# ImIntheMiddle/VATL4Pose-WACV2024

Measured on AMD Instinct MI355X. Metric: frames/sec pose-infer+uncertainty, 256x192 17-kp, higher is better.
Workload: dtype f32; 1 GPU; SimpleBaseline-R50 256x192 inference + decode + local-peak + THC-L1, 1024-frame synthetic video per GPU; frames_per_gpu=1024, batch=1024, tracks=4, parallelism=frame-sharded x1

## Files before the change

include/vatl_hip.h:

```cpp
#ifndef VATL_HIP_H
#define VATL_HIP_H

#include <stdint.h>

#ifdef __cplusplus
extern "C" {
#endif

#define VATL_VERSION 100
#define VATL_EINVAL  (-1)
#define VATL_ELAUNCH (-2)

int         vatl_version(void);
const char* vatl_last_error(void);

int vatl_flop_meter_begin(void);
int vatl_flop_meter_end(double* direct_flops, double* winograd_flops, int64_t* direct_launches, int64_t* winograd_launches);
#define VATL_ROUTE_NAMES "igemm,igemm_bnbwd,igemm_dma,persistent_1x1,streamk,rows_1x1,bottleneck_chain,stem_pool,halo_3x3," \
                         "winograd,winograd_2h,winograd_bnbwd,winograd_persist,winograd_c32,wgrad,winograd_wgrad,winograd_wgrad_2h," \
                         "winograd_wgrad_table,winograd_f4,winograd_f4_bnbwd,gemm1x1_ring,winograd_deconv43,winograd_s2_43,stem_pool_w1d," \
                         "chain_proj,chain_step,gemm1x1_bf16x6"
int vatl_flop_meter_routes(int64_t* counts, int n);


int vatl_nchw_to_nhwc(const float* src, float* dst, int N, int C, int H, int W, int Cpad, void* stream);
int vatl_nhwc_to_nchw(const float* src, float* dst, int N, int C, int H, int W, void* stream);

int vatl_pack_conv_weight(const float* w_oihw, float* w_packed, int Cout, int Cin, int R, int S,
                          int CoutPad, int Spad, int CinPad, void* stream);
int vatl_pack_deconv4x4s2_weight(const float* w_iohw, float* w_packed, int Cin, int Cout, int CoutPad, void* stream);
int64_t vatl_stem_pool_weight_floats(void);
int vatl_pack_stem_pool_weight(const float* w_oihw, float* packed, void* stream);
int vatl_stem_pool_supported(int H, int W);
int vatl_stem7x7s2_pool_fwd(const float* x_nchw, const float* w_packed, const float* scale, const float* bias, float* y_nhwc,
                            int N, int H, int W, void* stream);
int64_t vatl_stem_pool_w1d_weight_floats(void);
// ... 309 lines not shown
int vatl_deconv4x4s2_winograd43_supported(int N, int H, int W, int Cin, int Cout);
int vatl_deconv4x4s2_winograd43_fwd(const float* x, const float* u, const float* scale, const float* bias, float* y, int N, int H, int W,
                                    int Cin, int Cout, int relu, void* stream);
int64_t vatl_winograd_s2_43_weight_floats(int Cout, int Cin);
int vatl_pack_winograd_s2_43_weight(const float* w, float* u, int Cout, int Cin, void* stream);
int vatl_conv3x3s2_winograd43_supported(int N, int H, int W, int Cin, int Cout);
int vatl_conv3x3s2_winograd43_fwd(const float* x, const float* u, const float* scale, const float* bias, float* y, int N, int H, int W,
                                  int Cin, int Cout, int relu, void* stream);
int64_t vatl_gemm1x1_bf16x6_weight_floats(int N, int K);
int vatl_pack_gemm1x1_bf16x6_weight(const float* w, float* u, int N, int K, void* stream);
int vatl_gemm1x1_bf16x6_supported(int64_t M, int K, int K1, int N);
int vatl_gemm1x1_bf16x6_fwd(const float* x, const float* u, const float* scale, const float* bias, const float* residual, float* y,
                            int N, int H, int W, int Cin, int Cout, int stride, int relu, void* stream);
int vatl_gemm1x1_bf16x6_dual_fwd(const float* a, const float* x, const float* u, const float* bias, const float* residual, float* y,
                                 int N, int Ho, int Wo, int C1, int H2, int W2, int C2, int stride2, int Cout, int relu, void* stream);
int64_t vatl_winograd_deconv_stats_row_blocks(int64_t N, int H, int W);
int vatl_deconv4x4s2_winograd_fwd_stats(const float* x, const float* u, float* y, double* stats, int64_t* row_blocks_used, int N, int H, int W,
                                        int Cin, int Cout, void* stream);
int64_t vatl_conv3x3_winograd_wgrad_workspace_floats(int Cout, int Cin, int64_t N, int H, int W);
int vatl_conv3x3_winograd_wgrad(const float* x, const float* dz, float* dw, float* workspace, int N, int H, int W, int Cin, int Cout, void* stream);
int64_t vatl_deconv4x4s2_winograd_wgrad_workspace_floats(int Cin, int Cout, int64_t N, int H, int W);
int vatl_deconv4x4s2_winograd_wgrad(const float* x, const float* dy, float* dw, float* workspace, int N, int H, int W, int Cin, int Cout,
                                    void* stream);
int64_t vatl_winograd_deconv_dgrad_weight_floats(int Cin, int Cout);
int vatl_pack_winograd_deconv_dgrad_weight(const float* w, float* u, int Cin, int Cout, void* stream);
int vatl_deconv4x4s2_winograd_dgrad(const float* dz, const float* u, const float* residual, float* dx, int N, int H, int W, int Cin, int Cout,
                                    void* stream);
int vatl_deconv4x4s2_winograd_dgrad_bnbwd(const float* dz, const float* u, const float* residual, float* dx, int N, int H, int W, int Cin,
                                          int Cout, const float* bn_z, const float* bn_mask_y, const float* bn_scale, const float* bn_bias,
                                          const float* bn_mean, const float* bn_invstd, double* stats, int64_t* row_blocks_used, void* stream);
// ... 82 lines not shown
```

vatl4pose-wacv2024_amd/alphapose/models/hip_engine.py:

```python
from __future__ import annotations

import time
import weakref

import torch
import torch.nn as nn

import vatl_hip as vh

MAX_CHUNK = 1024



WINOGRAD = True
ROWS_GEMM = True
ROWS_GEMM_K = (128, 256)
WINO_C32 = True
WINO_F4 = True
DECONV_43 = True
S2_43 = True
BF16X6 = True


class _Conv:
    __slots__ = ("w", "u", "u32", "u4", "us2", "ux6", "wsrc", "wino", "c32", "f4", "s2", "x6", "scale", "bias", "cout", "r", "s", "stride", "pad")

    def __init__(self, conv: nn.Conv2d, bn: nn.BatchNorm2d | None):
        assert conv.groups == 1 and conv.dilation == (1, 1)
        assert conv.stride[0] == conv.stride[1] and conv.padding[0] == conv.padding[1]
        self.w = vh.pack_conv_weight(conv.weight.detach())
        self.cout, _, self.r, self.s = conv.weight.shape
        self.stride, self.pad = conv.stride[0], conv.padding[0]
        self.u = self.u32 = self.u4 = None
        self.wino = WINOGRAD and (self.r, self.s, self.stride, self.pad) == (3, 3, 1, 1) and conv.in_channels % 16 == 0 and self.cout % 4 == 0
        self.c32 = self.wino and WINO_C32 and conv.in_channels == 32 and self.cout == 32
        self.f4 = self.wino and WINO_F4 and conv.in_channels >= 64 and conv.in_channels % 16 == 0 and self.cout % 64 == 0
        self.us2 = None
        self.s2 = WINOGRAD and S2_43 and (self.r, self.s, self.stride, self.pad) == (3, 3, 2, 1) and conv.in_channels % 16 == 0 and self.cout % 64 == 0
        self.ux6 = None
        self.x6 = (BF16X6 and (self.r, self.s, self.stride, self.pad) == (1, 1, 1, 0) and conv.in_channels >= 512 and conv.in_channels % 64 == 0
                   and self.cout % 128 == 0)
        self.wsrc = conv.weight.detach() if self.wino or self.s2 else None
        cb =conv.bias.detach() if conv.bias is not None else None
        if bn is not None:
            self.scale, self.bias = vh.bn_fold(_d(bn.weight), _d(bn.bias), bn.running_mean, bn.running_var, bn.eps, cb)
        elif cb is not None:
            self.scale, self.bias = vh.bn_fold(None, None, None, None, 0.0, cb, channels=self.cout)
        else:
            self.scale = self.bias = None

    def __call__(self, x, relu, residual=None, out_nchw=False, out=None):
        if self.wino and not out_nchw and not vh.latency_mode():
            if self.c32 and vh.conv3x3_winograd_c32_supported(x.shape[0], x.shape[1], x.shape[2], 32, 32):
                if self.u32 is None:
                    self.u32 = vh.pack_winograd_c32_weight(self.wsrc)
                return vh.conv3x3_winograd_c32_fwd(x, self.u32, self.scale, self.bias, relu, residual=residual, out=out)
            if self.f4 and vh.conv3x3_winograd_f4_supported(x.shape[0], x.shape[1], x.shape[2], x.shape[3], self.cout):
                if self.u4 is None:
                    self.u4 = vh.pack_winograd_f4_weight(self.wsrc)
                return vh.conv3x3_winograd_f4_fwd(x, self.u4, self.scale, self.bias, self.cout, relu, residual=residual, out=out)
            if self.u is None:
                self.u = vh.pack_winograd_weight(self.wsrc)
            return vh.conv3x3_winograd_fwd(x, self.u, self.scale, self.bias, self.cout, relu, residual=residual, out=out)
        if (ROWS_GEMM and self.r == 1 and self.stride == 1 and not out_nchw and not vh.latency_mode() and x.shape[-1] in ROWS_GEMM_K
                and vh.conv1x1_rows_supported(x.shape[-1], 0, self.cout, x.shape[0] * x.shape[1] * x.shape[2])):
            return vh.conv1x1_rows_fwd(x, self.w, self.scale, self.bias, self.cout, relu, residual=residual, out=out)
        us2 = None
        if self.s2 and residual is None and not out_nchw and not vh.latency_mode():
            if self.us2 is None and vh.conv3x3s2_winograd43_supported(x.shape[0], x.shape[1], x.shape[2], x.shape[3], self.cout):
                self.us2 = vh.pack_winograd_s2_43_weight(self.wsrc)
            us2 = self.us2
        ux6 = None
        if self.x6 and not out_nchw and not vh.latency_mode():
            if self.ux6 is None and vh.gemm1x1_bf16x6_supported(x.shape[0] * x.shape[1] * x.shape[2], x.shape[3], 0, self.cout):
                self.ux6 = vh.pack_gemm1x1_bf16x6_weight(self.w)
            ux6 = self.ux6
        return vh.conv2d_fwd(x, self.w, self.scale, self.bias, self.cout, self.r, self.s, self.stride, self.pad, relu,
                             residual=residual, out_nchw=out_nchw, out=out, u_s2=us2, u_x6=ux6)
# ... 562 lines not shown
```

vatl4pose-wacv2024_amd/csrc/common.h:

```cpp
#pragma once
#include <hip/hip_runtime.h>
#include <atomic>
#include <cstdarg>
#include <cstdio>
#include <cstdint>

#include "vatl_hip.h"

namespace vatl {

char* err_buf();
int fail(int code, const char* fmt, ...);

void meter_add(int kind, double flops);
enum MeterRoute {
    kRouteIgemm = 0, kRouteIgemmBnBwd, kRouteIgemmDma, kRoutePersistent1x1, kRouteStreamK, kRouteRows, kRouteChain, kRouteStemPool, kRouteHalo,
    kRouteWino, kRouteWino2H, kRouteWinoBnBwd, kRouteWinoPersist, kRouteWinoC32, kRouteWgrad, kRouteWinoWgrad, kRouteWinoWgrad2H,
    kRouteWinoWgradTable, kRouteWinoF4, kRouteWinoF4BnBwd, kRouteGemm1x1Ring, kRouteWinoDeconv43, kRouteWinoS2_43, kRouteStemPoolW1d, kRouteChainProj,
    kRouteChainStep, kRouteGemm1x1Bf16x6, kRouteCount
};
void meter_route(int route);

inline int check_launch(const char* what) {
    hipError_t e = hipGetLastError();
    if (e != hipSuccess) return fail(VATL_ELAUNCH, "%s: %s", what, hipGetErrorString(e));
    return 0;
}

inline int ensure_dynamic_lds(const void* kern, int bytes, std::atomic<unsigned>& done_mask, const char* what) {
    int d = 0;
    if (hipGetDevice(&d) != hipSuccess) return fail(VATL_ELAUNCH, "%s: no current device", what);
    const unsigned bit = 1u << (d & 31);
    if (done_mask.load(std::memory_order_acquire) & bit) return 0;
    hipError_t e = hipFuncSetAttribute(kern, hipFuncAttributeMaxDynamicSharedMemorySize, bytes);
// ... 59 lines not shown
```

vatl4pose-wacv2024_amd/csrc/gemm1x1_bf16x6.hip:

```cpp
#include "conv_igemm.h"
#include "split16.h"
#include "tile_order.h"

namespace vatl {

constexpr int X6_BK = 16;
constexpr int X6_NS = 4;
constexpr int X6_A_FLOATS = 128 * X6_BK;
constexpr int X6_B_BYTES = 3 * 128 * X6_BK * 2;
constexpr int X6_STAGE = X6_A_FLOATS + X6_B_BYTES / 4;
constexpr int X6_BYTES = X6_NS * X6_STAGE * (int)sizeof(float);

typedef __bf16 x6_bf16x8 __attribute__((ext_vector_type(8)));

template <int N>
__device__ __forceinline__ void x6_wait_vm() {
    static_assert(N == 0 || N == 5 || N == 10, "add the count here");
    if constexpr (N == 0) asm volatile("s_waitcnt vmcnt(0)" ::: "memory");
    else if constexpr (N == 5) asm volatile("s_waitcnt vmcnt(5)" ::: "memory");
    else asm volatile("s_waitcnt vmcnt(10)" ::: "memory");
}

__device__ __forceinline__ f32x16 x6_mfma(u32x4 a, u32x4 b, f32x16 c) {
    return __builtin_amdgcn_mfma_f32_32x32x16_bf16(__builtin_bit_cast(x6_bf16x8, a), __builtin_bit_cast(x6_bf16x8, b), c, 0, 0, 0);
}

template <bool DUAL, bool RES>
__device__ __forceinline__ void gemm1x1_bf16x6_body(const ConvParams& p, float* smem) {
    const int tid = threadIdx.x, lane = tid & 63;
    const int wave = __builtin_amdgcn_readfirstlane(tid >> 6);
    const int wm = wave >> 1, wn = wave & 1;

    const int t = xcd_contiguous_index(blockIdx.x, gridDim.x);
    const int m_tile = t / p.n_tiles, n_tile = t - m_tile * p.n_tiles;
    const int m0 = m_tile * 128, n0 = n_tile * 128;

    const __amdgpu_buffer_rsrc_t xr = buf_rsrc(p.x, p.x_bytes);
    const __amdgpu_buffer_rsrc_t wr = buf_rsrc(p.w, p.w_bytes);
    const __amdgpu_buffer_rsrc_t xr2 = buf_rsrc(DUAL ? p.x2 : p.x, DUAL ? p.x2_bytes : p.x_bytes);

    const int S = p.ktiles * 2;
    const int S1 = DUAL ? p.k1 * 2 : S;

// ... 23 lines not shown
            if constexpr (DUAL && decltype(src)::value == 1) __builtin_amdgcn_raw_ptr_buffer_load_lds(xr2, da, 16, aoff2[u], (unsigned)(s - S1) * 64u, 0, 0);
            else                                             __builtin_amdgcn_raw_ptr_buffer_load_lds(xr, da, 16, aoff[u], (unsigned)s * 64u, 0, 0);
        }
#pragma unroll
        for (int u = 0; u < 3; ++u)
            __builtin_amdgcn_raw_ptr_buffer_load_lds(wr, (lds_void*)(st + X6_A_FLOATS + (4 * u + wave) * 256), 16, boff[u], (unsigned)s * (unsigned)X6_B_BYTES, 0, 0);
    };

    const int frow = lane & 31, h = lane >> 5;
    const int fsw = (frow >> 2) & 3;
    const float* Ard[2];
#pragma unroll
    for (int c = 0; c < 2; ++c) Ard[c] = smem + (wm * 64 + frow) * X6_BK + (((2 * h + c) ^ fsw) << 2);
    const float* Brd = smem + X6_A_FLOATS + (2 * wn * 64 + lane) * 4;

    f32x16 acc[2][2], sml[2][2];
#pragma unroll
    for (int i = 0; i < 2; ++i)
#pragma unroll
        for (int j = 0; j < 2; ++j)
#pragma unroll
            for (int e = 0; e < 16; ++e) { acc[i][j][e] = 0.f; sml[i][j][e] = 0.f; }

    auto stage = [&](auto slot, auto kind, auto src, int s) {
        constexpr int B = decltype(slot)::value, KIND = decltype(kind)::value;
        if constexpr (KIND <= 1) x6_wait_vm<10>();
        else if constexpr (KIND == 2) x6_wait_vm<5>();
        else x6_wait_vm<0>();
        __builtin_amdgcn_s_barrier();
        asm volatile("" ::: "memory");
        f32x4 af[2][2];
        u32x4 bw[3][2];
#pragma unroll
        for (int i = 0; i < 2; ++i)
#pragma unroll
            for (int c = 0; c < 2; ++c) af[i][c] = *reinterpret_cast<const f32x4*>(Ard[c] + B * X6_STAGE + i * 32 * X6_BK);
#pragma unroll
        for (int pl = 0; pl < 3; ++pl)
#pragma unroll
            for (int j = 0; j < 2; ++j) bw[pl][j] = *reinterpret_cast<const u32x4*>(Brd + B * X6_STAGE + (4 * pl + j) * 256);
        if constexpr (KIND == 0) issue(src, (B + 3) & 3, s + 3);
        u32x4 a0[2], a1[2], a2[2];
#pragma unroll
        for (int i = 0; i < 2; ++i)
#pragma unroll
            for (int d = 0; d < 4; ++d) {
                const split16::Pieces e = split16::split3(af[i][d >> 1][(2 * d) & 3]), o = split16::split3(af[i][d >> 1][(2 * d + 1) & 3]);
                a0[i][d] = split16::pack_pair(e.hi, o.hi);
                a1[i][d] = split16::pack_pair(e.mid, o.mid);
                a2[i][d] = split16::pack_pair(e.lo, o.lo);
            }
#pragma unroll
        for (int i = 0; i < 2; ++i)
#pragma unroll
            for (int j = 0; j < 2; ++j) acc[i][j] = x6_mfma(a0[i], bw[0][j], acc[i][j]);
#pragma unroll
// ... 37 lines not shown
    int s = 0;
    if constexpr (DUAL) {
        for (; s < S1 - 4; s += 4) group(C0{}, s);
        stage(C0{}, C0{}, C0{}, s);
        stage(C1{}, C0{}, X2{}, s + 1);
        stage(C2{}, C0{}, X2{}, s + 2);
        stage(C3{}, C0{}, X2{}, s + 3);
        s += 4;
    }
    for (; s < S - 4; s += 4) group(X2{}, s);
    stage(C0{}, C0{}, X2{}, s);
    stage(C1{}, C1{}, X2{}, s + 1);
    stage(C2{}, C2{}, X2{}, s + 2);
    stage(C3{}, C3{}, X2{}, s + 3);

    const unsigned rowb = (unsigned)p.Cout * 4u;
    const unsigned ylane = (unsigned)(m0 + wm * 64 + 4 * h) * rowb + (unsigned)(n0 + wn * 64 + frow) * 4u;
    const __amdgpu_buffer_rsrc_t yr = buf_rsrc(p.y, p.y_bytes);
    const __amdgpu_buffer_rsrc_t rr = buf_rsrc(RES ? p.res : p.y, RES ? p.y_bytes : 0u);
    float sc[2], bi[2];
#pragma unroll
    for (int j = 0; j < 2; ++j) {
        const int n = n0 + wn * 64 + j * 32 + frow;
        sc[j] = p.scale ? p.scale[n] : 1.f;
        bi[j] = p.bias ? p.bias[n] : 0.f;
    }
    const float lo = p.relu ? 0.f : -INFINITY;
#pragma unroll
    for (int i = 0; i < 2; ++i) {
        float rs[2][16];
#pragma unroll
        for (int j = 0; j < 2; ++j)
#pragma unroll
            for (int e = 0; e < 16; ++e)
                rs[j][e] = RES ? buf_load1(rr, ylane + (unsigned)(32 * i + (e & 3) + 8 * (e >> 2)) * rowb + (unsigned)j * 128u) : 0.f;
#pragma unroll
        for (int j = 0; j < 2; ++j)
#pragma unroll
            for (int e = 0; e < 16; ++e) {
                const float a = acc[i][j][e] + sml[i][j][e];
                const float v = fmaxf(a * sc[j] + bi[j] + rs[j][e], lo);
                buf_store1(yr, ylane + (unsigned)(32 * i + (e & 3) + 8 * (e >> 2)) * rowb + (unsigned)j * 128u, v);
            }
    }
}

template <bool DUAL, bool RES>
__global__ __launch_bounds__(256, 2) void gemm1x1_bf16x6_kernel(ConvParams p) {
    extern __shared__ __attribute__((aligned(16))) float smem[];
    gemm1x1_bf16x6_body<DUAL, RES>(p, smem);
}

__global__ __launch_bounds__(256) void gemm1x1_bf16x6_pack_kernel(const float* __restrict__ w, u32x4* __restrict__ u, int K, long long units) {
    const long long idx = (long long)blockIdx.x * 256 + threadIdx.x;
    if (idx >= units) return;
    const int S = K / X6_BK;
    const int l = (int)(idx & 63), jb = (int)((idx >> 6) & 3);
    const long long rest = idx >> 8;
    const int pl = (int)(rest % 3);
    const long long ts = rest / 3;
    const int st = (int)(ts % S), n_tile = (int)(ts / S);
    const float* src = w + (long long)(n_tile * 128 + jb * 32 + (l & 31)) * K + st * X6_BK + 8 * (l >> 5);
    float pc[8];
#pragma unroll
    for (int j = 0; j < 8; ++j) {
// ... 1 lines not shown
        pc[j] = pl == 0 ? q.hi : (pl == 1 ? q.mid : q.lo);
    }
    u32x4 o;
#pragma unroll
    for (int d = 0; d < 4; ++d) o[d] = split16::pack_pair(pc[2 * d], pc[2 * d + 1]);
    u[idx] = o;
}

static bool x6_shape_ok(long long M, int K, int K1, int N) {
    if (M < 1 || N < 128 || (N % 128) || K < 1 || (K % 64)) return false;
    if (K1 == 0 ? K < 512 : (K1 < 64 || (K1 % 64) || K - K1 < 64 || K < 384)) return false;
    if ((M + 128) * N >= (1LL << 30) || M * (K1 ? K1 : K) >= (1LL << 30) || 6LL * N * K >= (1LL << 31)) return false;
    return true;
}

template <bool DUAL, bool RES>
static int launch_x6_impl(const ConvParams& p, hipStream_t st) {
    auto kern = gemm1x1_bf16x6_kernel<DUAL, RES>;
    static std::atomic<unsigned> configured{0};
    if (int rc = ensure_dynamic_lds(reinterpret_cast<const void*>(kern), X6_BYTES, configured, "gemm1x1_bf16x6")) return rc;
    ConvParams q = p;
    q.n_tiles = p.Cout / 128;
    q.m_tiles = cdiv(p.M, 128);
    q.splits = 1;
    hipLaunchKernelGGL(kern, dim3((unsigned)(q.m_tiles * q.n_tiles)), dim3(256), X6_BYTES, st, q);
    meter_add(0, (6.0 / 16.0) * 2.0 * ((double)q.m_tiles * 128) * ((double)q.n_tiles * 128) * ((double)q.ktiles * BK));
    meter_route(kRouteGemm1x1Bf16x6);
    return check_launch("gemm1x1_bf16x6");
}

}

using namespace vatl;

extern "C" int64_t vatl_gemm1x1_bf16x6_weight_floats(int N, int K) { return 3LL * N * K / 2; }

extern "C" int vatl_pack_gemm1x1_bf16x6_weight(const float* w, float* u, int N, int K, void* stream) {
    if (!w || !u) return fail(VATL_EINVAL, "pack_gemm1x1_bf16x6_weight: null pointer");
    if (N < 128 || (N % 128) || K < 64 || (K % 64) || 6LL * N * K >= (1LL << 31))
        return fail(VATL_EINVAL, "pack_gemm1x1_bf16x6_weight: N %d must be a multiple of 128, K %d of 64, 6 N K below 2^31 bytes", N, K);
    const long long units = 6LL * N * K / 16;
    hipLaunchKernelGGL(gemm1x1_bf16x6_pack_kernel, dim3((unsigned)((units + 255) / 256)), dim3(256), 0, (hipStream_t)stream, w, reinterpret_cast<u32x4*>(u), K, units);
    return check_launch("gemm1x1_bf16x6_pack");
}

extern "C" int vatl_gemm1x1_bf16x6_supported(int64_t M, int K, int K1, int N) { return x6_shape_ok(M, K, K1, N) ? 1 : 0; }

extern "C" int vatl_gemm1x1_bf16x6_fwd(const float* x, const float* u, const float* scale, const float* bias, const float* residual, float* y,
                                       int N, int H, int W, int Cin, int Cout, int stride, int relu, void* stream) {
    if (!x || !u || !y || N <= 0 || H <= 0 || W <= 0) return fail(VATL_EINVAL, "gemm1x1_bf16x6_fwd: null pointer or empty batch");
    const long long M = (long long)N * H * W;
    if (stride != 1 || !x6_shape_ok(M, Cin, 0, Cout))
        return fail(VATL_EINVAL, "gemm1x1_bf16x6_fwd: %lld x %d -> %d, stride %d is outside stride 1, K %% 64 == 0, K >= 512, N %% 128 == 0 and 32-bit offsets", M, Cin, Cout, stride);
    ConvParams p{};
    p.x = x; p.w = u; p.scale = scale; p.bias = bias; p.res = residual; p.y = y;
    p.N = N; p.H = H; p.W = W; p.Cin = Cin; p.Cout = Cout; p.CoutPad = Cout;
    p.R = 1; p.S = 1; p.stride = 1;
    p.Ho = H; p.Wo = W; p.M = (int)M;
    p.OH = H; p.OW = W; p.osy = 1; p.osx = 1;
    p.relu = relu;
    p.kpr = Cin / BK; p.ktiles = p.kpr; p.K = Cin;
    p.x_bytes = (unsigned)(M * Cin * 4); p.y_bytes = (unsigned)(M * Cout * 4); p.w_bytes = (unsigned)(6LL * Cout * Cin);
    p.d_HoWo = make_fastdiv((unsigned)(H * W)); p.d_Wo = make_fastdiv((unsigned)W);
    return residual ? launch_x6_impl<false, true>(p, (hipStream_t)stream) : launch_x6_impl<false, false>(p, (hipStream_t)stream);
}

extern "C" int vatl_gemm1x1_bf16x6_dual_fwd(const float* a, const float* x, const float* u, const float* bias, const float* residual, float* y,
                                            int N, int Ho, int Wo, int C1, int H2, int W2, int C2, int stride2, int Cout, int relu, void* stream) {
    if (!a || !x || !u || !y || N <= 0 || Ho <= 0 || Wo <= 0) return fail(VATL_EINVAL, "gemm1x1_bf16x6_dual_fwd: null pointer or empty batch");
    if (residual) return fail(VATL_EINVAL, "gemm1x1_bf16x6_dual_fwd: the dual form takes no residual");
    if (stride2 < 1 || (long long)(Ho - 1) * stride2 >= H2 || (long long)(Wo - 1) * stride2 >= W2)
        return fail(VATL_EINVAL, "gemm1x1_bf16x6_dual_fwd: stride %d does not map %dx%d onto %dx%d", stride2, Ho, Wo, H2, W2);
    const long long M = (long long)N * Ho * Wo, x2e = (long long)N * H2 * W2 * C2;
    if (C1 <= 0 || C2 <= 0 || !x6_shape_ok(M, C1 + C2, C1, Cout) || x2e >= (1LL << 30))
        return fail(VATL_EINVAL, "gemm1x1_bf16x6_dual_fwd: %lld x (%d + %d) -> %d is outside C1 %% 64 == 0, C2 %% 64 == 0, K >= 384, N %% 128 == 0 and 32-bit offsets", M, C1, C2, Cout);
    ConvParams p{};
    p.x = a; p.x2 = x; p.w = u; p.bias = bias; p.y = y;
    p.N = N; p.H = Ho; p.W = Wo; p.Cin = C1; p.Cout = Cout; p.CoutPad = Cout;
    p.R = 1; p.S = 1; p.stride = 1;
// ... 10 lines not shown
```

vatl4pose-wacv2024_amd/vatl_hip/__init__.py:

```python
from __future__ import annotations

import ctypes as C
import os
import threading as _threading

import torch

_HERE = os.path.dirname(os.path.abspath(__file__))
LIB_PATH = os.environ.get("VATL_HIP_LIB") or os.path.join(_HERE, "libvatl_hip.so")

_p = C.c_void_p
_i = C.c_int
_f = C.c_float
_d = C.c_double
_i64 = C.c_int64

SIGNATURES = {
    "vatl_version": (_i, []),
    "vatl_last_error": (C.c_char_p, []),
    "vatl_flop_meter_begin": (_i, []),
    "vatl_flop_meter_end": (_i, [_p, _p, _p, _p]),
    "vatl_flop_meter_routes": (_i, [_p, _i]),
    "vatl_nchw_to_nhwc": (_i, [_p, _p, _i, _i, _i, _i, _i, _p]),
    "vatl_nhwc_to_nchw": (_i, [_p, _p, _i, _i, _i, _i, _p]),
# ... 94 lines not shown
    "vatl_pack_winograd_deconv_weight": (_i, [_p, _p, _i, _i, _p]),
    "vatl_deconv4x4s2_winograd_fwd": (_i, [_p] * 5 + [_i] * 6 + [_p]),
    "vatl_winograd_deconv43_weight_floats": (_i64, [_i, _i]),
    "vatl_pack_winograd_deconv43_weight": (_i, [_p, _p, _i, _i, _p]),
    "vatl_deconv4x4s2_winograd43_supported": (_i, [_i, _i, _i, _i, _i]),
    "vatl_deconv4x4s2_winograd43_fwd": (_i, [_p] * 5 + [_i] * 6 + [_p]),
    "vatl_winograd_s2_43_weight_floats": (_i64, [_i, _i]),
    "vatl_pack_winograd_s2_43_weight": (_i, [_p, _p, _i, _i, _p]),
    "vatl_conv3x3s2_winograd43_supported": (_i, [_i, _i, _i, _i, _i]),
    "vatl_conv3x3s2_winograd43_fwd": (_i, [_p] * 5 + [_i] * 6 + [_p]),
    "vatl_gemm1x1_bf16x6_weight_floats": (_i64, [_i, _i]),
    "vatl_pack_gemm1x1_bf16x6_weight": (_i, [_p, _p, _i, _i, _p]),
    "vatl_gemm1x1_bf16x6_supported": (_i, [_i64, _i, _i, _i]),
    "vatl_gemm1x1_bf16x6_fwd": (_i, [_p] * 6 + [_i] * 7 + [_p]),
    "vatl_gemm1x1_bf16x6_dual_fwd": (_i, [_p] * 6 + [_i] * 10 + [_p]),
    "vatl_winograd_deconv_stats_row_blocks": (_i64, [_i64, _i, _i]),
    "vatl_deconv4x4s2_winograd_fwd_stats": (_i, [_p, _p, _p, _p, _p, _i, _i, _i, _i, _i, _p]),
    "vatl_conv2d_fwd_stats": (_i, [_p, _p, _p, _p, _p, _i, _i, _i, _i, _i, _i, _i, _i, _i, _i, _p]),
    "vatl_deconv4x4s2_fwd_stats": (_i, [_p, _p, _p, _p, _p, _i, _i, _i, _i, _i, _i, _p]),
    "vatl_bn_train_finalize": (_i, [_p, _i64, _i64, _i, _p, _p, _p, _p, _f, _f, _p, _p, _p, _p, _p]),
    "vatl_maxpool3x3s2_bwd": (_i, [_p, _p, _p, _i, _i, _i, _i, _p]),
    "vatl_maxpool3x3s2_fwd_idx": (_i, [_p, _p, _p, _i, _i, _i, _i, _p]),
    "vatl_pack_weights_multi": (_i, [_p, _i, _i64, _p]),
    "vatl_adamw_multi_block_elems": (_i64, []),
    "vatl_checksum_block_words": (_i64, []),
    "vatl_checksum_multi": (_i, [_p, _i, _i64, _p, _p]),
    "vatl_maxpool3x3s2_fwd_idx_affine": (_i, [_p, _p, _p, _p, _p, _i, _i, _i, _i, _p]),
    "vatl_bn_train_bwd_relu_pool": (_i, [_p, _p, _p, _p, _p, _p, _p, _p, _p, _p, _p, _i, _i, _i, _i, _p, _p, _p]),
    "vatl_maxpool3x3s2_bwd_idx": (_i, [_p, _p, _p, _i, _i, _i, _i, _p]),
    "vatl_pixelunshuffle2": (_i, [_p, _p, _i, _i, _i, _i, _p]),
# ... 156 lines not shown
    y = torch.empty((n, h, w, cpad), device=x.device, dtype=torch.float32)
    _check(lib().vatl_nchw_to_nhwc(_ptr(x), _ptr(y), n, c, h, w, cpad, _stream()), "vatl_nchw_to_nhwc")
    return y


def nhwc_to_nchw(x: torch.Tensor) -> torch.Tensor:
    n, h, w, c = x.shape
    y = torch.empty((n, c, h, w), device=x.device, dtype=torch.float32)
    _check(lib().vatl_nhwc_to_nchw(_ptr(x), _ptr(y), n, c, h, w, _stream()), "vatl_nhwc_to_nchw")
    return y



ROUTE_NAMES = ("igemm", "igemm_bnbwd", "igemm_dma", "persistent_1x1", "streamk", "rows_1x1", "bottleneck_chain", "stem_pool", "halo_3x3", "winograd",
               "winograd_2h", "winograd_bnbwd", "winograd_persist", "winograd_c32", "wgrad", "winograd_wgrad", "winograd_wgrad_2h", "winograd_wgrad_table", "winograd_f4", "winograd_f4_bnbwd",
               "gemm1x1_ring", "winograd_deconv43", "winograd_s2_43", "stem_pool_w1d", "chain_proj", "chain_step", "gemm1x1_bf16x6")


class flop_meter:

    def __enter__(self):
        _check(lib().vatl_flop_meter_begin(), "flop_meter_begin")
        self.direct = self.winograd = self.total = 0.0
        self.direct_launches = self.winograd_launches = 0
        return self

    @staticmethod
    def launches_now() -> int:
        counts = (C.c_int64 * len(ROUTE_NAMES))()
        _check(min(0, lib().vatl_flop_meter_routes(counts, len(ROUTE_NAMES))), "flop_meter_routes")
        return int(sum(counts))
# ... 352 lines not shown
    scale = torch.empty(c, device=dev, dtype=torch.float32)
    bias = torch.empty(c, device=dev, dtype=torch.float32)
    _check(lib().vatl_bn_fold(_ptr(gamma), _ptr(beta), _ptr(mean), _ptr(var), _ptr(conv_bias), eps, _ptr(scale), _ptr(bias), c, _stream()), "vatl_bn_fold")
    return scale, bias



def conv3x3s2_winograd43_supported(n: int, h: int, w: int, cin: int, cout: int) -> bool:
    return bool(lib().vatl_conv3x3s2_winograd43_supported(n, h, w, cin, cout))


def gemm1x1_bf16x6_supported(m: int, k: int, k1: int, n: int) -> bool:
    return bool(lib().vatl_gemm1x1_bf16x6_supported(m, k, k1, n))


def conv2d_fwd(x, w_packed, scale, bias, cout: int, r: int, s: int, stride: int, pad: int, relu: bool,
               residual=None, out_nchw: bool = False, out=None, u_s2=None, u_x6=None):
    n, h, w, cin = x.shape
    ho = (h + 2 * pad - r) // stride + 1
    wo = (w + 2 * pad - s) // stride + 1
    shape = (n, cout, ho, wo) if out_nchw else (n, ho, wo, cout)
    y = out if out is not None else torch.empty(shape, device=x.device, dtype=torch.float32)
    if (u_s2 is not None and (r, s, stride, pad) == (3, 3, 2, 1) and residual is None and not out_nchw
            and conv3x3s2_winograd43_supported(n, h, w, cin, cout)):
        _check(lib().vatl_conv3x3s2_winograd43_fwd(_ptr(x), _ptr(u_s2), _ptr(scale), _ptr(bias), _ptr(y), n, h, w, cin, cout, int(relu), _stream()),
               "vatl_conv3x3s2_winograd43_fwd")
        return y
    if u_x6 is not None and (r, s, stride, pad) == (1, 1, 1, 0) and not out_nchw and gemm1x1_bf16x6_supported(n * h * w, cin, 0, cout):
        _check(lib().vatl_gemm1x1_bf16x6_fwd(_ptr(x), _ptr(u_x6), _ptr(scale), _ptr(bias), _ptr(residual), _ptr(y), n, h, w, cin, cout, stride, int(relu),
                                             _stream()), "vatl_gemm1x1_bf16x6_fwd")
# ... 8 lines not shown
    _, h2, w2, c2 = x.shape
    y = out if out is not None else torch.empty((n, ho, wo, cout), device=a.device, dtype=torch.float32)
    if u_x6 is not None and gemm1x1_bf16x6_supported(n * ho * wo, c1 + c2, c1, cout):
        _check(lib().vatl_gemm1x1_bf16x6_dual_fwd(_ptr(a), _ptr(x), _ptr(u_x6), _ptr(bias), None, _ptr(y), n, ho, wo, c1, h2, w2, c2, stride2, cout, int(relu),
                                                  _stream()), "vatl_gemm1x1_bf16x6_dual_fwd")
        return y
    _check(lib().vatl_conv1x1_dual_fwd(_ptr(a), _ptr(x), _ptr(w_packed), _ptr(bias), _ptr(y), n, ho, wo, c1, h2, w2, c2, stride2, cout,
                                       w_packed.shape[0], int(relu), _stream()), "vatl_conv1x1_dual_fwd")
    return y


def conv1x1_rows_supported(k1: int, k2: int, n: int, m: int) -> bool:
    return bool(lib().vatl_conv1x1_rows_supported(k1, k2, n, m))


def conv1x1_rows_fwd(a, w, scale, bias, cout: int, relu: bool, residual=None, x2=None, out=None, next_conv1=None, y1_out=None):
    n, h, w_, k1 = a.shape
    k2 = 0 if x2 is None else x2.shape[-1]
    assert w.numel() >= cout * (k1 + k2) and (x2 is None or tuple(x2.shape[:3]) == (n, h, w_)) and (residual is None or tuple(residual.shape) == (n, h, w_, cout))
    y = out if out is not None else torch.empty((n, h, w_, cout), device=a.device, dtype=torch.float32)
    assert a.is_contiguous() and y.is_contiguous() and (x2 is None or x2.is_contiguous()) and (residual is None or residual.is_contiguous())
    if next_conv1 is not None:
        w1, scale1, bias1 = next_conv1
        cnext = w1.shape[0]
        if x2 is None or k2 != k1 or residual is not None:
            raise VatlError("conv1x1_rows_fwd: next_conv1 goes with the two-source form (a, x2 of 64 channels each) and no residual")
        assert w1.numel() == cnext * cout
        y1 = y1_out if y1_out is not None else torch.empty((n, h, w_, cnext), device=a.device, dtype=torch.float32)
        assert y1.is_contiguous()
        _check(lib().vatl_chain_proj_fwd(_ptr(a), _ptr(x2), _ptr(w), _ptr(scale), _ptr(bias), _ptr(y), _ptr(w1), _ptr(scale1), _ptr(bias1), _ptr(y1),
                                         n * h * w_, k1, cout, cnext, int(relu), _stream()), "vatl_chain_proj_fwd")
        return y, y1
    _check(lib().vatl_conv1x1_rows_fwd(_ptr(a), _ptr(x2), _ptr(w), _ptr(scale), _ptr(bias), _ptr(residual), _ptr(y), n * h * w_, k1, k2, cout, int(relu),
                                       _stream()), "vatl_conv1x1_rows_fwd")
    return y


def bottleneck_chain_supported(cmid: int, cout: int, cnext: int, m: int) -> bool:
    return bool(lib().vatl_bottleneck_chain_supported(cmid, cout, cnext, m))


def chain_proj_supported(cmid: int, cout: int, cnext: int, m: int) -> bool:
    return bool(lib().vatl_chain_proj_supported(cmid, cout, cnext, m))


def chain_step_supported(cmid: int, cout: int, cnext: int, m: int) -> bool:
    return bool(lib().vatl_chain_step_supported(cmid, cout, cnext, m))
# ... 1739 lines not shown
```

Baseline: 18990 frames/s.

## Add short-K bf16x6 MFMA 1x1 GEMM route with LDS-staged residual epilogue

Adds a short-K variant of the split-bf16 (bf16x6) MFMA 1x1 conv kernel for K in [256,512) with Cout >= 512, and routes matching expand convs (for example 256->1024 in ResNet-50 stage 3) to it instead of the FP32 rows GEMM. The residual tile is prefetched into LDS with buffer_load_lds during the tail pipeline stages, so the epilogue reads it from LDS rather than issuing scattered global loads. This aims to move short-K 1x1 convs onto matrix cores and hide residual-read latency. The cost is extra synchronisation, added LDS use and bf16x6 emulation overhead, which can weigh more when K is short.

```diff
diff --git a/include/vatl_hip.h b/include/vatl_hip.h
--- a/include/vatl_hip.h
+++ b/include/vatl_hip.h
@@ -19,7 +19,7 @@
 #define VATL_ROUTE_NAMES "igemm,igemm_bnbwd,igemm_dma,persistent_1x1,streamk,rows_1x1,bottleneck_chain,stem_pool,halo_3x3," \
                          "winograd,winograd_2h,winograd_bnbwd,winograd_persist,winograd_c32,wgrad,winograd_wgrad,winograd_wgrad_2h," \
                          "winograd_wgrad_table,winograd_f4,winograd_f4_bnbwd,gemm1x1_ring,winograd_deconv43,winograd_s2_43,stem_pool_w1d," \
-                         "chain_proj,chain_step,gemm1x1_bf16x6"
+                         "chain_proj,chain_step,gemm1x1_bf16x6,gemm1x1_bf16x6_short"
 int vatl_flop_meter_routes(int64_t* counts, int n);
 
 
@@ -359,6 +359,9 @@
                             int N, int H, int W, int Cin, int Cout, int stride, int relu, void* stream);
 int vatl_gemm1x1_bf16x6_dual_fwd(const float* a, const float* x, const float* u, const float* bias, const float* residual, float* y,
                                  int N, int Ho, int Wo, int C1, int H2, int W2, int C2, int stride2, int Cout, int relu, void* stream);
+int vatl_gemm1x1_bf16x6_short_supported(int64_t M, int K, int N);
+int vatl_gemm1x1_bf16x6_short_fwd(const float* x, const float* u, const float* scale, const float* bias, const float* residual, float* y,
+                                  int N, int H, int W, int Cin, int Cout, int stride, int relu, void* stream);
 int64_t vatl_winograd_deconv_stats_row_blocks(int64_t N, int H, int W);
 int vatl_deconv4x4s2_winograd_fwd_stats(const float* x, const float* u, float* y, double* stats, int64_t* row_blocks_used, int N, int H, int W,
                                         int Cin, int Cout, void* stream);
diff --git a/vatl4pose-wacv2024_amd/alphapose/models/hip_engine.py b/vatl4pose-wacv2024_amd/alphapose/models/hip_engine.py
--- a/vatl4pose-wacv2024_amd/alphapose/models/hip_engine.py
+++ b/vatl4pose-wacv2024_amd/alphapose/models/hip_engine.py
@@ -20,10 +20,12 @@
 DECONV_43 = True
 S2_43 = True
 BF16X6 = True
+BF16X6_SHORT = True
+BF16X6_SHORT_MIN_K = 256
 
 
 class _Conv:
-    __slots__ = ("w", "u", "u32", "u4", "us2", "ux6", "wsrc", "wino", "c32", "f4", "s2", "x6", "scale", "bias", "cout", "r", "s", "stride", "pad")
+    __slots__ = ("w", "u", "u32", "u4", "us2", "ux6", "wsrc", "wino", "c32", "f4", "s2", "x6", "x6s", "scale", "bias", "cout", "r", "s", "stride", "pad")
 
     def __init__(self, conv: nn.Conv2d, bn: nn.BatchNorm2d | None):
         assert conv.groups == 1 and conv.dilation == (1, 1)
@@ -40,6 +42,8 @@
         self.ux6 = None
         self.x6 = (BF16X6 and (self.r, self.s, self.stride, self.pad) == (1, 1, 1, 0) and conv.in_channels >= 512 and conv.in_channels % 64 == 0
                    and self.cout % 128 == 0)
+        self.x6s = (BF16X6 and BF16X6_SHORT and (self.r, self.s, self.stride, self.pad) == (1, 1, 1, 0) and max(128, BF16X6_SHORT_MIN_K) <= conv.in_channels < 512
+                    and conv.in_channels % 64 == 0 and self.cout >= 512 and self.cout % 256 == 0)
         self.wsrc = conv.weight.detach() if self.wino or self.s2 else None
         cb =conv.bias.detach() if conv.bias is not None else None
         if bn is not None:
@@ -62,6 +66,10 @@
             if self.u is None:
                 self.u = vh.pack_winograd_weight(self.wsrc)
             return vh.conv3x3_winograd_fwd(x, self.u, self.scale, self.bias, self.cout, relu, residual=residual, out=out)
+        if self.x6s and not out_nchw and not vh.latency_mode() and vh.gemm1x1_bf16x6_short_supported(x.shape[0] * x.shape[1] * x.shape[2], x.shape[3], self.cout):
+            if self.ux6 is None:
+                self.ux6 = vh.pack_gemm1x1_bf16x6_weight(self.w)
+            return vh.conv1x1_rows_fwd(x, self.w, self.scale, self.bias, self.cout, relu, residual=residual, out=out, u_x6=self.ux6)
         if (ROWS_GEMM and self.r == 1 and self.stride == 1 and not out_nchw and not vh.latency_mode() and x.shape[-1] in ROWS_GEMM_K
                 and vh.conv1x1_rows_supported(x.shape[-1], 0, self.cout, x.shape[0] * x.shape[1] * x.shape[2])):
             return vh.conv1x1_rows_fwd(x, self.w, self.scale, self.bias, self.cout, relu, residual=residual, out=out)
diff --git a/vatl4pose-wacv2024_amd/csrc/common.h b/vatl4pose-wacv2024_amd/csrc/common.h
--- a/vatl4pose-wacv2024_amd/csrc/common.h
+++ b/vatl4pose-wacv2024_amd/csrc/common.h
@@ -17,7 +17,7 @@
     kRouteIgemm = 0, kRouteIgemmBnBwd, kRouteIgemmDma, kRoutePersistent1x1, kRouteStreamK, kRouteRows, kRouteChain, kRouteStemPool, kRouteHalo,
     kRouteWino, kRouteWino2H, kRouteWinoBnBwd, kRouteWinoPersist, kRouteWinoC32, kRouteWgrad, kRouteWinoWgrad, kRouteWinoWgrad2H,
     kRouteWinoWgradTable, kRouteWinoF4, kRouteWinoF4BnBwd, kRouteGemm1x1Ring, kRouteWinoDeconv43, kRouteWinoS2_43, kRouteStemPoolW1d, kRouteChainProj,
-    kRouteChainStep, kRouteGemm1x1Bf16x6, kRouteCount
+    kRouteChainStep, kRouteGemm1x1Bf16x6, kRouteGemm1x1Bf16x6Short, kRouteCount
 };
 void meter_route(int route);
 
diff --git a/vatl4pose-wacv2024_amd/csrc/gemm1x1_bf16x6.hip b/vatl4pose-wacv2024_amd/csrc/gemm1x1_bf16x6.hip
--- a/vatl4pose-wacv2024_amd/csrc/gemm1x1_bf16x6.hip
+++ b/vatl4pose-wacv2024_amd/csrc/gemm1x1_bf16x6.hip
@@ -25,8 +25,16 @@
     return __builtin_amdgcn_mfma_f32_32x32x16_bf16(__builtin_bit_cast(x6_bf16x8, a), __builtin_bit_cast(x6_bf16x8, b), c, 0, 0, 0);
 }
 
-template <bool DUAL, bool RES>
+struct X6Epilogue {
+    unsigned rowb, ylane;
+    __amdgpu_buffer_rsrc_t yr, rr;
+    float sc[2], bi[2], lo;
+};
+
+template <bool DUAL, bool RES, bool SHORT = false>
 __device__ __forceinline__ void gemm1x1_bf16x6_body(const ConvParams& p, float* smem) {
+    static_assert(!(SHORT && DUAL), "the short-K form is plain");
+    constexpr bool LDSRES = SHORT && RES;
     const int tid = threadIdx.x, lane = tid & 63;
     const int wave = __builtin_amdgcn_readfirstlane(tid >> 6);
     const int wm = wave >> 1, wn = wave & 1;
@@ -80,6 +88,44 @@
     for (int c = 0; c < 2; ++c) Ard[c] = smem + (wm * 64 + frow) * X6_BK + (((2 * h + c) ^ fsw) << 2);
     const float* Brd = smem + X6_A_FLOATS + (2 * wn * 64 + lane) * 4;
 
+    auto epilogue_operands = [&]() {
+        X6Epilogue ep;
+        ep.rowb = (unsigned)p.Cout * 4u;
+        ep.ylane = (unsigned)(m0 + wm * 64 + 4 * h) * ep.rowb + (unsigned)(n0 + wn * 64 + frow) * 4u;
+        ep.yr = buf_rsrc(p.y, p.y_bytes);
+        ep.rr = buf_rsrc(RES ? p.res : p.y, RES ? p.y_bytes : 0u);
+#pragma unroll
+        for (int j = 0; j < 2; ++j) {
+            const int n = n0 + wn * 64 + j * 32 + frow;
+            ep.sc[j] = p.scale ? p.scale[n] : 1.f;
+            ep.bi[j] = p.bias ? p.bias[n] : 0.f;
+        }
+        ep.lo = p.relu ? 0.f : -INFINITY;
+        return ep;
+    };
+    X6Epilogue ep;
+    if constexpr (SHORT) ep = epilogue_operands();
+    float dres[2][4];
+    unsigned roff = 0;
+    if constexpr (LDSRES) {
+#pragma unroll
+        for (int j = 0; j < 2; ++j)
+#pragma unroll
+            for (int r = 0; r < 4; ++r) dres[j][r] = buf_load1(ep.rr, ep.ylane + (unsigned)(56 + r) * ep.rowb + (unsigned)j * 128u);
+        roff = (unsigned)n0 * 4u + (unsigned)((lane & 31) ^ ((wave >> 1) << 3)) * 16u;
+    }
+    const int rrow = m0 + 2 * wave + (lane >> 5);
+    auto issue_res = [&](auto piece) {
+        constexpr int Q = decltype(piece)::value;
+#pragma unroll
+        for (int u = 0; u < (Q < 2 ? 5 : 4); ++u) {
+            const int cr0 = 40 * Q + 8 * u;
+            const int row0 = cr0 + (cr0 >= 56 ? 8 : 0);
+            __builtin_amdgcn_raw_ptr_buffer_load_lds(ep.rr, (lds_void*)(smem + (20 * Q + 4 * u + wave) * 256), 16,
+                                                     (unsigned)min(rrow + row0, p.M - 1) * ep.rowb + roff, 0, 0, 0);
+        }
+    };
+
     f32x16 acc[2][2], sml[2][2];
 #pragma unroll
     for (int i = 0; i < 2; ++i)
@@ -90,7 +136,7 @@
 
     auto stage = [&](auto slot, auto kind, auto src, int s) {
         constexpr int B = decltype(slot)::value, KIND = decltype(kind)::value;
-        if constexpr (KIND <= 1) x6_wait_vm<10>();
+        if constexpr (KIND <= 1 || LDSRES) x6_wait_vm<10>();
         else if constexpr (KIND == 2) x6_wait_vm<5>();
         else x6_wait_vm<0>();
         __builtin_amdgcn_s_barrier();
@@ -106,6 +152,7 @@
 #pragma unroll
             for (int j = 0; j < 2; ++j) bw[pl][j] = *reinterpret_cast<const u32x4*>(Brd + B * X6_STAGE + (4 * pl + j) * 256);
         if constexpr (KIND == 0) issue(src, (B + 3) & 3, s + 3);
+        else if constexpr (LDSRES) issue_res(std::integral_constant<int, KIND - 1>{});
         u32x4 a0[2], a1[2], a2[2];
 #pragma unroll
         for (int i = 0; i < 2; ++i)
@@ -173,34 +220,62 @@
     stage(C2{}, C2{}, X2{}, s + 2);
     stage(C3{}, C3{}, X2{}, s + 3);
 
-    const unsigned rowb = (unsigned)p.Cout * 4u;
-    const unsigned ylane = (unsigned)(m0 + wm * 64 + 4 * h) * rowb + (unsigned)(n0 + wn * 64 + frow) * 4u;
-    const __amdgpu_buffer_rsrc_t yr = buf_rsrc(p.y, p.y_bytes);
-    const __amdgpu_buffer_rsrc_t rr = buf_rsrc(RES ? p.res : p.y, RES ? p.y_bytes : 0u);
-    float sc[2], bi[2];
-#pragma unroll
-    for (int j = 0; j < 2; ++j) {
-        const int n = n0 + wn * 64 + j * 32 + frow;
-        sc[j] = p.scale ? p.scale[n] : 1.f;
-        bi[j] = p.bias ? p.bias[n] : 0.f;
-    }
-    const float lo = p.relu ? 0.f : -INFINITY;
-#pragma unroll
-    for (int i = 0; i < 2; ++i) {
-        float rs[2][16];
-#pragma unroll
-        for (int j = 0; j < 2; ++j)
-#pragma unroll
-            for (int e = 0; e < 16; ++e)
-                rs[j][e] = RES ? buf_load1(rr, ylane + (unsigned)(32 * i + (e & 3) + 8 * (e >> 2)) * rowb + (unsigned)j * 128u) : 0.f;
-#pragma unroll
-        for (int j = 0; j < 2; ++j)
-#pragma unroll
-            for (int e = 0; e < 16; ++e) {
-                const float a = acc[i][j][e] + sml[i][j][e];
-                const float v = fmaxf(a * sc[j] + bi[j] + rs[j][e], lo);
-                buf_store1(yr, ylane + (unsigned)(32 * i + (e & 3) + 8 * (e >> 2)) * rowb + (unsigned)j * 128u, v);
-            }
+    if constexpr (!SHORT) {
+        const unsigned rowb = (unsigned)p.Cout * 4u;
+        const unsigned ylane = (unsigned)(m0 + wm * 64 + 4 * h) * rowb + (unsigned)(n0 + wn * 64 + frow) * 4u;
+        const __amdgpu_buffer_rsrc_t yr = buf_rsrc(p.y, p.y_bytes);
+        const __amdgpu_buffer_rsrc_t rr = buf_rsrc(RES ? p.res : p.y, RES ? p.y_bytes : 0u);
+        float sc[2], bi[2];
+#pragma unroll
+        for (int j = 0; j < 2; ++j) {
+            const int n = n0 + wn * 64 + j * 32 + frow;
+            sc[j] = p.scale ? p.scale[n] : 1.f;
+            bi[j] = p.bias ? p.bias[n] : 0.f;
+        }
+        const float lo = p.relu ? 0.f : -INFINITY;
+#pragma unroll
+        for (int i = 0; i < 2; ++i) {
+            float rs[2][16];
+#pragma unroll
+            for (int j = 0; j < 2; ++j)
+#pragma unroll
+                for (int e = 0; e < 16; ++e)
+                    rs[j][e] = RES ? buf_load1(rr, ylane + (unsigned)(32 * i + (e & 3) + 8 * (e >> 2)) * rowb + (unsigned)j * 128u) : 0.f;
+#pragma unroll
+            for (int j = 0; j < 2; ++j)
+#pragma unroll
+                for (int e = 0; e < 16; ++e) {
+                    const float a = acc[i][j][e] + sml[i][j][e];
+                    const float v = fmaxf(a * sc[j] + bi[j] + rs[j][e], lo);
+                    buf_store1(yr, ylane + (unsigned)(32 * i + (e & 3) + 8 * (e >> 2)) * rowb + (unsigned)j * 128u, v);
+                }
+        }
+    } else {
+        if constexpr (RES) {
+            x6_wait_vm<0>();
+            __builtin_amdgcn_s_barrier();
+            asm volatile("" ::: "memory");
+        }
+        const float* resL = smem + (wm * 56 + 4 * h) * 128 + wn * 64 + frow;
+#pragma unroll
+        for (int i = 0; i < 2; ++i) {
+            float rs[2][16];
+#pragma unroll
+            for (int j = 0; j < 2; ++j)
+#pragma unroll
+                for (int e = 0; e < 16; ++e) {
+                    if constexpr (!RES) rs[j][e] = 0.f;
+                    else rs[j][e] = (i == 1 && e >= 12) ? dres[j][e - 12] : resL[(32 * i + (e & 3) + 8 * (e >> 2)) * 128 + ((j ^ h) << 5)];
+                }
+#pragma unroll
+            for (int j = 0; j < 2; ++j)
+#pragma unroll
+                for (int e = 0; e < 16; ++e) {
+                    const float a = acc[i][j][e] + sml[i][j][e];
+                    const float v = fmaxf(a * ep.sc[j] + ep.bi[j] + rs[j][e], ep.lo);
+                    buf_store1(ep.yr, ep.ylane + (unsigned)(32 * i + (e & 3) + 8 * (e >> 2)) * ep.rowb + (unsigned)j * 128u, v);
+                }
+        }
     }
 }
 
@@ -208,6 +283,12 @@
 __global__ __launch_bounds__(256, 2) void gemm1x1_bf16x6_kernel(ConvParams p) {
     extern __shared__ __attribute__((aligned(16))) float smem[];
     gemm1x1_bf16x6_body<DUAL, RES>(p, smem);
+}
+
+template <bool RES>
+__global__ __launch_bounds__(256, 2) void gemm1x1_bf16x6_short_kernel(ConvParams p) {
+    extern __shared__ __attribute__((aligned(16))) float smem[];
+    gemm1x1_bf16x6_body<false, RES, true>(p, smem);
 }
 
 __global__ __launch_bounds__(256) void gemm1x1_bf16x6_pack_kernel(const float* __restrict__ w, u32x4* __restrict__ u, int K, long long units) {
@@ -239,19 +320,28 @@
     return true;
 }
 
-template <bool DUAL, bool RES>
+static bool x6_short_shape_ok(long long M, int K, int N) {
+    if (M < 1 || N < 512 || (N % 256) || K < 128 || K >= 512 || (K % 64)) return false;
+    if ((M + 128) * N >= (1LL << 30) || M * K >= (1LL << 30) || 6LL * N * K >= (1LL << 31)) return false;
+    return true;
+}
+
+template <bool DUAL, bool RES, bool SHORT = false>
 static int launch_x6_impl(const ConvParams& p, hipStream_t st) {
-    auto kern = gemm1x1_bf16x6_kernel<DUAL, RES>;
+    auto kern = [] {
+        if constexpr (SHORT) return gemm1x1_bf16x6_short_kernel<RES>;
+        else return gemm1x1_bf16x6_kernel<DUAL, RES>;
+    }();
     static std::atomic<unsigned> configured{0};
-    if (int rc = ensure_dynamic_lds(reinterpret_cast<const void*>(kern), X6_BYTES, configured, "gemm1x1_bf16x6")) return rc;
+    if (int rc = ensure_dynamic_lds(reinterpret_cast<const void*>(kern), X6_BYTES, configured, SHORT ? "gemm1x1_bf16x6_short" : "gemm1x1_bf16x6")) return rc;
     ConvParams q = p;
     q.n_tiles = p.Cout / 128;
     q.m_tiles = cdiv(p.M, 128);
     q.splits = 1;
     hipLaunchKernelGGL(kern, dim3((unsigned)(q.m_tiles * q.n_tiles)), dim3(256), X6_BYTES, st, q);
     meter_add(0, (6.0 / 16.0) * 2.0 * ((double)q.m_tiles * 128) * ((double)q.n_tiles * 128) * ((double)q.ktiles * BK));
-    meter_route(kRouteGemm1x1Bf16x6);
-    return check_launch("gemm1x1_bf16x6");
+    meter_route(SHORT ? kRouteGemm1x1Bf16x6Short : kRouteGemm1x1Bf16x6);
+    return check_launch(SHORT ? "gemm1x1_bf16x6_short" : "gemm1x1_bf16x6");
 }
 
 }
@@ -269,14 +359,9 @@
     return check_launch("gemm1x1_bf16x6_pack");
 }
 
-extern "C" int vatl_gemm1x1_bf16x6_supported(int64_t M, int K, int K1, int N) { return x6_shape_ok(M, K, K1, N) ? 1 : 0; }
-
-extern "C" int vatl_gemm1x1_bf16x6_fwd(const float* x, const float* u, const float* scale, const float* bias, const float* residual, float* y,
-                                       int N, int H, int W, int Cin, int Cout, int stride, int relu, void* stream) {
-    if (!x || !u || !y || N <= 0 || H <= 0 || W <= 0) return fail(VATL_EINVAL, "gemm1x1_bf16x6_fwd: null pointer or empty batch");
+static ConvParams x6_plain_params(const float* x, const float* u, const float* scale, const float* bias, const float* residual, float* y,
+                                  int N, int H, int W, int Cin, int Cout, int relu) {
     const long long M = (long long)N * H * W;
-    if (stride != 1 || !x6_shape_ok(M, Cin, 0, Cout))
-        return fail(VATL_EINVAL, "gemm1x1_bf16x6_fwd: %lld x %d -> %d, stride %d is outside stride 1, K %% 64 == 0, K >= 512, N %% 128 == 0 and 32-bit offsets", M, Cin, Cout, stride);
     ConvParams p{};
     p.x = x; p.w = u; p.scale = scale; p.bias = bias; p.res = residual; p.y = y;
     p.N = N; p.H = H; p.W = W; p.Cin = Cin; p.Cout = Cout; p.CoutPad = Cout;
@@ -287,7 +372,31 @@
     p.kpr = Cin / BK; p.ktiles = p.kpr; p.K = Cin;
     p.x_bytes = (unsigned)(M * Cin * 4); p.y_bytes = (unsigned)(M * Cout * 4); p.w_bytes = (unsigned)(6LL * Cout * Cin);
     p.d_HoWo = make_fastdiv((unsigned)(H * W)); p.d_Wo = make_fastdiv((unsigned)W);
+    return p;
+}
+
+extern "C" int vatl_gemm1x1_bf16x6_supported(int64_t M, int K, int K1, int N) { return x6_shape_ok(M, K, K1, N) ? 1 : 0; }
+
+extern "C" int vatl_gemm1x1_bf16x6_fwd(const float* x, const float* u, const float* scale, const float* bias, const float* residual, float* y,
+                                       int N, int H, int W, int Cin, int Cout, int stride, int relu, void* stream) {
+    if (!x || !u || !y || N <= 0 || H <= 0 || W <= 0) return fail(VATL_EINVAL, "gemm1x1_bf16x6_fwd: null pointer or empty batch");
+    const long long M = (long long)N * H * W;
+    if (stride != 1 || !x6_shape_ok(M, Cin, 0, Cout))
+        return fail(VATL_EINVAL, "gemm1x1_bf16x6_fwd: %lld x %d -> %d, stride %d is outside stride 1, K %% 64 == 0, K >= 512, N %% 128 == 0 and 32-bit offsets", M, Cin, Cout, stride);
+    const ConvParams p = x6_plain_params(x, u, scale, bias, residual, y, N, H, W, Cin, Cout, relu);
     return residual ? launch_x6_impl<false, true>(p, (hipStream_t)stream) : launch_x6_impl<false, false>(p, (hipStream_t)stream);
+}
+
+extern "C" int vatl_gemm1x1_bf16x6_short_supported(int64_t M, int K, int N) { return x6_short_shape_ok(M, K, N) ? 1 : 0; }
+
+extern "C" int vatl_gemm1x1_bf16x6_short_fwd(const float* x, const float* u, const float* scale, const float* bias, const float* residual, float* y,
+                                             int N, int H, int W, int Cin, int Cout, int stride, int relu, void* stream) {
+    if (!x || !u || !y || N <= 0 || H <= 0 || W <= 0) return fail(VATL_EINVAL, "gemm1x1_bf16x6_short_fwd: null pointer or empty batch");
+    const long long M = (long long)N * H * W;
+    if (stride != 1 || !x6_short_shape_ok(M, Cin, Cout))
+        return fail(VATL_EINVAL, "gemm1x1_bf16x6_short_fwd: %lld x %d -> %d, stride %d is outside stride 1, K %% 64 == 0, 128 <= K < 512, N %% 256 == 0, N >= 512 and 32-bit offsets", M, Cin, Cout, stride);
+    const ConvParams p = x6_plain_params(x, u, scale, bias, residual, y, N, H, W, Cin, Cout, relu);
+    return residual ? launch_x6_impl<false, true, true>(p, (hipStream_t)stream) : launch_x6_impl<false, false, true>(p, (hipStream_t)stream);
 }
 
 extern "C" int vatl_gemm1x1_bf16x6_dual_fwd(const float* a, const float* x, const float* u, const float* bias, const float* residual, float* y,
diff --git a/vatl4pose-wacv2024_amd/vatl_hip/__init__.py b/vatl4pose-wacv2024_amd/vatl_hip/__init__.py
--- a/vatl4pose-wacv2024_amd/vatl_hip/__init__.py
+++ b/vatl4pose-wacv2024_amd/vatl_hip/__init__.py
@@ -132,6 +132,8 @@
     "vatl_gemm1x1_bf16x6_supported": (_i, [_i64, _i, _i, _i]),
     "vatl_gemm1x1_bf16x6_fwd": (_i, [_p] * 6 + [_i] * 7 + [_p]),
     "vatl_gemm1x1_bf16x6_dual_fwd": (_i, [_p] * 6 + [_i] * 10 + [_p]),
+    "vatl_gemm1x1_bf16x6_short_supported": (_i, [_i64, _i, _i]),
+    "vatl_gemm1x1_bf16x6_short_fwd": (_i, [_p] * 6 + [_i] * 7 + [_p]),
     "vatl_winograd_deconv_stats_row_blocks": (_i64, [_i64, _i, _i]),
     "vatl_deconv4x4s2_winograd_fwd_stats": (_i, [_p, _p, _p, _p, _p, _i, _i, _i, _i, _i, _p]),
     "vatl_conv2d_fwd_stats": (_i, [_p, _p, _p, _p, _p, _i, _i, _i, _i, _i, _i, _i, _i, _i, _i, _p]),
@@ -318,7 +320,8 @@
 
 ROUTE_NAMES = ("igemm", "igemm_bnbwd", "igemm_dma", "persistent_1x1", "streamk", "rows_1x1", "bottleneck_chain", "stem_pool", "halo_3x3", "winograd",
                "winograd_2h", "winograd_bnbwd", "winograd_persist", "winograd_c32", "wgrad", "winograd_wgrad", "winograd_wgrad_2h", "winograd_wgrad_table", "winograd_f4", "winograd_f4_bnbwd",
-               "gemm1x1_ring", "winograd_deconv43", "winograd_s2_43", "stem_pool_w1d", "chain_proj", "chain_step", "gemm1x1_bf16x6")
+               "gemm1x1_ring", "winograd_deconv43", "winograd_s2_43", "stem_pool_w1d", "chain_proj", "chain_step", "gemm1x1_bf16x6",
+               "gemm1x1_bf16x6_short")
 
 
 class flop_meter:
@@ -701,6 +704,10 @@
     return bool(lib().vatl_gemm1x1_bf16x6_supported(m, k, k1, n))
 
 
+def gemm1x1_bf16x6_short_supported(m: int, k: int, n: int) -> bool:
+    return bool(lib().vatl_gemm1x1_bf16x6_short_supported(m, k, n))
+
+
 def conv2d_fwd(x, w_packed, scale, bias, cout: int, r: int, s: int, stride: int, pad: int, relu: bool,
                residual=None, out_nchw: bool = False, out=None, u_s2=None, u_x6=None):
     n, h, w, cin = x.shape
@@ -739,7 +746,7 @@
     return bool(lib().vatl_conv1x1_rows_supported(k1, k2, n, m))
 
 
-def conv1x1_rows_fwd(a, w, scale, bias, cout: int, relu: bool, residual=None, x2=None, out=None, next_conv1=None, y1_out=None):
+def conv1x1_rows_fwd(a, w, scale, bias, cout: int, relu: bool, residual=None, x2=None, out=None, next_conv1=None, y1_out=None, u_x6=None):
     n, h, w_, k1 = a.shape
     k2 = 0 if x2 is None else x2.shape[-1]
     assert w.numel() >= cout * (k1 + k2) and (x2 is None or tuple(x2.shape[:3]) == (n, h, w_)) and (residual is None or tuple(residual.shape) == (n, h, w_, cout))
@@ -756,6 +763,10 @@
         _check(lib().vatl_chain_proj_fwd(_ptr(a), _ptr(x2), _ptr(w), _ptr(scale), _ptr(bias), _ptr(y), _ptr(w1), _ptr(scale1), _ptr(bias1), _ptr(y1),
                                          n * h * w_, k1, cout, cnext, int(relu), _stream()), "vatl_chain_proj_fwd")
         return y, y1
+    if u_x6 is not None and x2 is None and gemm1x1_bf16x6_short_supported(n * h * w_, k1, cout):
+        _check(lib().vatl_gemm1x1_bf16x6_short_fwd(_ptr(a), _ptr(u_x6), _ptr(scale), _ptr(bias), _ptr(residual), _ptr(y), n, h, w_, k1, cout, 1, int(relu),
+                                                   _stream()), "vatl_gemm1x1_bf16x6_short_fwd")
+        return y
     _check(lib().vatl_conv1x1_rows_fwd(_ptr(a), _ptr(x2), _ptr(w), _ptr(scale), _ptr(bias), _ptr(residual), _ptr(y), n * h * w_, k1, k2, cout, int(relu),
                                        _stream()), "vatl_conv1x1_rows_fwd")
     return y
```

New measurement: 19420 frames/s, median of 6. 2.3% higher.
